# ERGO-Code/ipx

Hardware: AMD Instinct MI355X
Metric: kkt_solves_per_sec (higher is better)
Workload: dtype f64; 1 GPU; C3 synthetic LP m=1000000 n=2000000 8 nnz/col (nnz=16000000), KKTSolverDiag::Solve = diag-precond CR to tol=0.3*sqrt(mu), scaling spread s=1; rows of AI partitioned over 1 GPU(s); errflag=0

## Files before the change

### ipx_amd/csrc/cr.hip

```cpp
#include <cmath>

#include "context.hpp"
#include "spmv_kernels.hpp"

namespace ipxk {

constexpr int kWindow = 2;

enum CrMode { kModePcrDiag = 0, kModePcrSmw = 1, kModePlain = 2 };

struct CrVecs {
    int m;
    double* lhs;
    double* residual;
    double* sresidual;
    double* step;
    double* Cstep;
    double* Cres;
    double* pCstep;
    const double* resscale;
    const double* diag;
};

__global__ __launch_bounds__(kBlock) void residual_init_kernel(int m, const double* __restrict__ rhs,
                                                               const double* __restrict__ sub,
                                                               const double* __restrict__ resscale,
                                                               double* __restrict__ out,
                                                               double* partial) {
    __shared__ double red[kBlock / 64 + 1];
    double mx = 0.0;
    for (int i = blockIdx.x * kBlock + threadIdx.x; i < m; i += gridDim.x * kBlock) {
        const double r = sub ? rhs[i] - sub[i] : rhs[i];
        out[i] = r;
        mx = MaxOp::apply(mx, fabs(resscale ? resscale[i] * r : r));
    }
    mx = block_reduce<MaxOp>(mx, red);
    if (threadIdx.x == 0) partial[blockIdx.x] = mx;
}

__global__ __launch_bounds__(kBlock) void cr_init_state_kernel(CrState* st, double tol, long long maxiter,
                                                               long long hist_cap, PartRef rsdot, int mode) {
    __shared__ double red[kBlock / 64 + 1];
    const double r = rsdot.p ? reduce_partials<SumOp>(rsdot, red) : 0.0;
    if (threadIdx.x == 0) {
        st->tol = tol;
        st->maxiter = maxiter;
        st->k_started = 0;
        st->k_finished = 0;
        st->cdot[0] = st->cdot[1] = 0.0;
        st->rps[0] = r;
        st->rps[1] = 0.0;
        st->resnorm = 0.0;
        st->iter = 0;
        st->errflag = 0;
        st->done = 0;
        st->hist_cap = hist_cap;
        st->diag_rps_old = st->diag_rps_new = 0.0;
        st->mode = mode;
    }
}

template <int MODE>
__global__ __launch_bounds__(kBlock) void cr_control_update_kernel(
    CrState* st, CrVecs v, PartRef res0, PartRef res1, PartRef pdot_ref, PartRef rsdot_ref,
    double* res_next0, double* res_next1, double* hist) {
    if (st->done) return;
    __shared__ double red[kBlock / 64 + 1];
    const long long k = st->k_finished;
    const bool writer = blockIdx.x == 0 && threadIdx.x == 0;
    int errflag = -1;
    double resnorm = st->resnorm;

    if (MODE != kModePlain && k > 0 && k % 5 == 0) {
        const double rsdot = reduce_partials<SumOp>(rsdot_ref, red);
        const long long c5 = k / 5;
        if (rsdot >= st->rps[(c5 - 1) & 1]) {
            errflag = 204;
            if (writer) { st->diag_rps_old = st->rps[(c5 - 1) & 1]; st->diag_rps_new = rsdot; }
        } else if (writer) st->rps[c5 & 1] = rsdot;
    }
    double alpha = 0.0;
    if (errflag < 0) {
        resnorm = reduce_partials<MaxOp>((k & 1) ? res1 : res0, red);
        if (writer && k < st->hist_cap) hist[k] = resnorm;
        const double cdot = st->cdot[k & 1];
        if (resnorm <= st->tol) errflag = 0;
        else if (k == st->maxiter) errflag = 201;
        else if (cdot <= 0.0) errflag = 202;
        else {
            const double pdot = reduce_partials<SumOp>(pdot_ref, red);
            if (MODE != kModePlain && pdot <= 0.0) errflag = 203;
            else {
                alpha = cdot / pdot;
                if (!isfinite(alpha)) errflag = 205;
            }
        }
    }
    if (errflag >= 0) {
        if (writer) {
            st->errflag = errflag;
            st->iter = k;
            st->resnorm = resnorm;
            st->done = 1;
        }
        return;
    }

    double mx = 0.0;
    for (int i = blockIdx.x * kBlock + threadIdx.x; i < v.m; i += gridDim.x * kBlock) {
        const double q = v.Cstep[i];
        v.lhs[i] += alpha * v.step[i];
        const double r = v.residual[i] - alpha * q;
        v.residual[i] = r;
        if (MODE == kModePcrDiag) v.sresidual[i] -= alpha * (q / v.diag[i]);
        if (MODE == kModePcrSmw) v.sresidual[i] -= alpha * v.pCstep[i];
        mx = MaxOp::apply(mx, fabs(v.resscale ? v.resscale[i] * r : r));
    }
    mx = block_reduce<MaxOp>(mx, red);
    if (threadIdx.x == 0) ((k & 1) ? res_next0 : res_next1)[blockIdx.x] = mx;
    if (writer) {
        st->k_started = k + 1;
        st->resnorm = resnorm;
    }
}

template <int MODE, bool INIT>
__global__ __launch_bounds__(kBlock) void cr_direction_kernel(CrState* st, CrVecs v, PartRef cdot_ref,
                                                              double* pdot_partial) {
    if (st->done) return;
    __shared__ double red[kBlock / 64 + 1];
    const long long k = INIT ? -1 : st->k_started - 1;
    const double cdotnew = reduce_partials<SumOp>(cdot_ref, red);
    const double beta = INIT ? 0.0 : cdotnew / st->cdot[k & 1];
    const double* src = MODE == kModePlain ? v.residual : v.sresidual;
    double acc = 0.0;
    for (int i = blockIdx.x * kBlock + threadIdx.x; i < v.m; i += gridDim.x * kBlock) {
        double p, q;
        if (INIT) {
            p = src[i];
            q = v.Cres[i];
        } else {
            p = src[i] + beta * v.step[i];
            q = v.Cres[i] + beta * v.Cstep[i];
        }
        v.step[i] = p;
        v.Cstep[i] = q;
        if (MODE == kModePcrDiag) acc += (q / v.diag[i]) * q;
        if (MODE == kModePlain) acc += q * q;
    }
    if (MODE != kModePcrSmw) {
        acc = block_reduce<SumOp>(acc, red);
        if (threadIdx.x == 0) pdot_partial[blockIdx.x] = acc;
    }
    if (blockIdx.x == 0 && threadIdx.x == 0) {
        st->cdot[(k + 1) & 1] = cdotnew;
        st->k_finished = k + 1;
    }
}

__global__ __launch_bounds__(kBlock) void finalize_scalar_kernel(PartRef ref, int op, double* out) {
    __shared__ double red[kBlock / 64 + 1];
    const double v = op == 1 ? reduce_partials<MaxOp>(ref, red)
                   : op == 2 ? reduce_partials<MinOp>(ref, red) : reduce_partials<SumOp>(ref, red);
    if (threadIdx.x == 0) *out = v;
}

__global__ void snapshot_done_kernel(const CrState* st, int* host_slot) {
    __hip_atomic_store(host_slot, st->done, __ATOMIC_RELAXED, __HIP_MEMORY_SCOPE_SYSTEM);
}
__global__ void cycle_flags_kernel(const CrState* st, double interrupt_flag, double* flags) {
    flags[0] = (double)st->done;
    flags[1] = interrupt_flag;
}
__global__ void snapshot_flags_kernel(const double* flags, int* host_done, int* host_interrupt) {
    __hip_atomic_store(host_interrupt, (int)flags[1], __ATOMIC_RELAXED, __HIP_MEMORY_SCOPE_SYSTEM);
    __hip_atomic_store(host_done, (int)flags[0], __ATOMIC_RELAXED, __HIP_MEMORY_SCOPE_SYSTEM);
}

constexpr int kDoneRing = kWindow + 2;

static void ensure_comm_buffers(Context* c) {
    if (c->comm_scalars.size() < 64) c->comm_scalars.resize(64);
    if (c->comm_send.size() < (size_t)kNumPartialSlots) {
        c->comm_send.resize(kNumPartialSlots);
        IPXK_HIP(hipMemsetAsync(c->comm_send.get(), 0, sizeof(double) * kNumPartialSlots, c->stream));
    }
    const size_t need = (size_t)c->nranks * kNumPartialSlots;
    if (c->comm_gather.size() < need) c->comm_gather.resize(need);
}

struct Pub {
    Context* c;
    bool multi;
    explicit Pub(Context* ctx) : c(ctx), multi(comm_rows(ctx)) { if (multi) ensure_comm_buffers(ctx); }
    PartRef ref(int slot, int nparts) const {
        if (!multi) return PartRef{c->part(slot), nparts, 1};
        return PartRef{c->comm_gather.get() + slot, c->nranks, kNumPartialSlots};
    }
    void publish(int slot0, int n0, int op0, int slot1 = -1, int n1 = 0, int op1 = 0) const {
        if (!multi) return;
        hipLaunchKernelGGL(finalize_scalar_kernel, dim3(1), dim3(kBlock), 0, c->stream,
                           PartRef{c->part(slot0), n0, 1}, op0, c->comm_send.get() + slot0);
        if (slot1 >= 0)
            hipLaunchKernelGGL(finalize_scalar_kernel, dim3(1), dim3(kBlock), 0, c->stream,
                               PartRef{c->part(slot1), n1, 1}, op1, c->comm_send.get() + slot1);
        comm_allgather(c, c->comm_send.get(), c->comm_gather.get(), kNumPartialSlots);
    }
};

PartRef publish_scalar(Context* c, int slot, int count, int op) {
    const Pub pub(c);
    pub.publish(slot, count, op);
    return pub.ref(slot, count);
}

PartRef allreduce_scalar(Context* c, int slot, int count, int op) {
    ensure_comm_buffers(c);
    double* out = c->comm_scalars.get() + 62;
    hipLaunchKernelGGL(finalize_scalar_kernel, dim3(1), dim3(kBlock), 0, c->stream,
                       PartRef{c->part(slot), count, 1}, op, out);
    if (op == 0) comm_allreduce_sum(c, out, 1);
    else if (op == 1) comm_allreduce_max(c, out, 1);
    else comm_allreduce_min(c, out, 1);
    return PartRef{out, 1, 1};
}

double reduce_partials_host(Context* c, int slot, int count, bool is_max) {
    ensure_comm_buffers(c);
    double* out = c->comm_scalars.get() + 63;
    hipLaunchKernelGGL(finalize_scalar_kernel, dim3(1), dim3(kBlock), 0, c->stream,
                       PartRef{c->part(slot), count, 1}, is_max ? 1 : 0, out);
    if (comm_rows(c)) {
        if (is_max) comm_allreduce_max(c, out, 1);
        else comm_allreduce_sum(c, out, 1);
    }
    double v = 0.0;
    IPXK_HIP(hipMemcpyAsync(&v, out, sizeof(double), hipMemcpyDeviceToHost, c->stream));
    IPXK_HIP(hipStreamSynchronize(c->stream));
    return v;
}

static void ensure_workspaces(Context* c) {
    const size_t m = (size_t)(c->m > 0 ? c->m : 1);
    if (c->v_residual.size() != m) {
        c->v_residual.resize(m); c->v_sresidual.resize(m); c->v_step.resize(m);
        c->v_Cstep.resize(m); c->v_Cres.resize(m); c->v_pCstep.resize(m);
    }
    if (c->partials.size() == 0) c->partials.resize((size_t)kNumPartialSlots * kPartialStride);
    if (c->state.size() == 0) c->state.resize(1);
    if (!c->h_state) IPXK_HIP(hipHostMalloc(reinterpret_cast<void**>(&c->h_state), sizeof(CrState)));
    if (!c->ev_a) { IPXK_HIP(hipEventCreate(&c->ev_a)); IPXK_HIP(hipEventCreate(&c->ev_b)); }
    if (!c->h_cycle_done) {
        IPXK_HIP(hipHostMalloc(reinterpret_cast<void**>(&c->h_cycle_done), 64 * sizeof(int), hipHostMallocMapped));
        IPXK_HIP(hipHostGetDevicePointer(reinterpret_cast<void**>(&c->d_cycle_done), c->h_cycle_done, 0));
    }
    while ((int)c->ev_window.size() < kWindow + 1) {
        hipEvent_t e;
        IPXK_HIP(hipEventCreateWithFlags(&e, hipEventDisableTiming));
        c->ev_window.push_back(e);
    }
}

struct CrOps {
    int mode;
    int (*applyC)(Context*, const double* rhs, double* lhs, const int* done);
};

static int applyC_normal(Context* c, const double* rhs, double* lhs, const int* done) {
    int np = 0;
    time_mark(c, kTimeOp, true);
    normal_apply_dev(c, c->W, rhs, lhs, &np, done);
    time_mark(c, kTimeOp, false);
    return np;
}
static int applyC_split(Context* c, const double* rhs, double* lhs, const int* done) {
    return split_apply_dev(c, rhs, lhs, done);
}

template <int MODE>
static CrResult run_cr(Context* c, const CrOps& ops, const double* rhs, double tol,
                       const double* resscale, ipxint maxiter, double* lhs, bool lhs_is_zero,
                       ipxk_interrupt_fn interrupt, void* user, double* hist_host, ipxint hist_cap,
                       ipxk_times* times) {
    ensure_workspaces(c);
    time_start(c, times);
    hipStream_t s = c->stream;
    const int m = (int)c->m;
    if (maxiter < 0) maxiter = (comm_active(c) ? c->m_global : c->m) + 100;
    if (hist_cap < 0) hist_cap = 0;
    if (!hist_host) hist_cap = 0;
    if (c->hist.size() < (size_t)hist_cap + 1) c->hist.resize((size_t)hist_cap + 1);
    CrState* st = c->state.get();
    int* done = &st->done;
    const int g = vec_grid(m);
    const Pub pub(c);
    for (int i = 0; i < 2 * kDoneRing; i++) c->h_cycle_done[i] = 0;
    const bool multi = comm_active(c);
    if (multi) ensure_comm_buffers(c);

    CrVecs v;
    v.m = m; v.lhs = lhs; v.residual = c->v_residual.get(); v.sresidual = c->v_sresidual.get();
    v.step = c->v_step.get(); v.Cstep = c->v_Cstep.get(); v.Cres = c->v_Cres.get();
    v.pCstep = c->v_pCstep.get(); v.resscale = resscale; v.diag = c->reord.in_use ? c->reord.diagonal.get() : c->diagonal.get();

    IPXK_HIP(hipEventRecord(c->ev_a, s));

    if (lhs_is_zero) {
        hipLaunchKernelGGL(residual_init_kernel, dim3(g), dim3(kBlock), 0, s, m, rhs,
                           (const double*)nullptr, resscale, v.residual, c->part(kPartRes0));
    } else {
        ops.applyC(c, lhs, v.Cres, nullptr);
        hipLaunchKernelGGL(residual_init_kernel, dim3(g), dim3(kBlock), 0, s, m, rhs,
                           (const double*)v.Cres, resscale, v.residual, c->part(kPartRes0));
    }
    int nrsdot = 0;
    if (MODE != kModePlain) nrsdot = diag_apply_dev(c, v.residual, v.sresidual, kPartRsdot, nullptr);
    if (MODE != kModePlain) pub.publish(kPartRes0, g, 1, kPartRsdot, nrsdot, 0);
    else pub.publish(kPartRes0, g, 1);
    const PartRef res0 = pub.ref(kPartRes0, g), res1 = pub.ref(kPartRes1, g);
    const PartRef rsdot = MODE != kModePlain ? pub.ref(kPartRsdot, nrsdot) : PartRef{nullptr, 0, 1};
    hipLaunchKernelGGL(cr_init_state_kernel, dim3(1), dim3(kBlock), 0, s, st, tol, (long long)maxiter,
                       (long long)hist_cap, rsdot, (int)MODE);
    const double* csrc = MODE == kModePlain ? v.residual : v.sresidual;
    int ncdot = ops.applyC(c, csrc, v.Cres, nullptr);
    pub.publish(kPartCdot, ncdot, 0);
    hipLaunchKernelGGL((cr_direction_kernel<MODE, true>), dim3(g), dim3(kBlock), 0, s, st, v,
                       pub.ref(kPartCdot, ncdot), c->part(kPartPdot));
    int npdot = g;
    if (MODE == kModePcrSmw) npdot = diag_apply_dev(c, v.Cstep, v.pCstep, kPartPdot, nullptr);
    pub.publish(kPartPdot, npdot, 0);
    const PartRef pdot_ref = pub.ref(kPartPdot, npdot);

    ipxint interrupt_flag = 0, my_interrupt = 0;
    bool agreed_done = false;
    for (long long cycle = 0;; cycle++) {
        const long long k0 = cycle * 5;
        if (k0 > maxiter) break;
        if (cycle >= kWindow) {
            const long long cw = cycle - kWindow;
            IPXK_HIP(hipEventSynchronize(c->ev_window[cw % (kWindow + 1)]));
            if (*(volatile int*)(c->h_cycle_done + cw % kDoneRing)) { agreed_done = true; break; }
            if (multi) {
                const int agreed = *(volatile int*)(c->h_cycle_done + kDoneRing + cw % kDoneRing);
                if (agreed != 0) { interrupt_flag = agreed; break; }
            }
        }
        if (interrupt && cycle > 0) {
            my_interrupt = interrupt(user);
            if (!multi && my_interrupt != 0) { interrupt_flag = my_interrupt; break; }
        }
        for (long long k = k0; k < k0 + 5 && k <= maxiter; k++) {
            hipLaunchKernelGGL((cr_control_update_kernel<MODE>), dim3(g), dim3(kBlock), 0, s, st, v,
                               res0, res1, pdot_ref, rsdot, c->part(kPartRes0), c->part(kPartRes1),
                               c->hist.get());
            ncdot = ops.applyC(c, csrc, v.Cres, done);
            pub.publish(kPartCdot, ncdot, 0, ((k + 1) & 1) ? kPartRes1 : kPartRes0, g, 1);
            hipLaunchKernelGGL((cr_direction_kernel<MODE, false>), dim3(g), dim3(kBlock), 0, s, st, v,
                               pub.ref(kPartCdot, ncdot), c->part(kPartPdot));
            if (MODE == kModePcrSmw) diag_apply_dev(c, v.Cstep, v.pCstep, kPartPdot, done);
            if (MODE != kModePlain && (k + 1) % 5 == 0) {
                diag_apply_dev(c, v.residual, v.sresidual, kPartRsdot, done);
                pub.publish(kPartPdot, npdot, 0, kPartRsdot, nrsdot, 0);
            } else {
                pub.publish(kPartPdot, npdot, 0);
            }
        }
        if (multi) {
            double* flags = c->comm_scalars.get() + 56;
            hipLaunchKernelGGL(cycle_flags_kernel, dim3(1), dim3(1), 0, s, st, (double)my_interrupt, flags);
            comm_allreduce_max(c, flags, 2);
            hipLaunchKernelGGL(snapshot_flags_kernel, dim3(1), dim3(1), 0, s, flags, c->d_cycle_done + cycle % kDoneRing,
                               c->d_cycle_done + kDoneRing + cycle % kDoneRing);
        } else {
            hipLaunchKernelGGL(snapshot_done_kernel, dim3(1), dim3(1), 0, s, st, c->d_cycle_done + cycle % kDoneRing);
        }
        IPXK_HIP(hipEventRecord(c->ev_window[cycle % (kWindow + 1)], s));
    }
    IPXK_HIP(hipEventRecord(c->ev_b, s));
    IPXK_HIP(hipMemcpyAsync(c->h_state, st, sizeof(CrState), hipMemcpyDeviceToHost, s));
    IPXK_HIP(hipStreamSynchronize(s));
    IPXK_HIP(hipGetLastError());
    comm_check(c);

    if (multi && agreed_done && !c->h_state->done)
        throw Error(IPXK_E_HIP, "ranks of a partitioned solve diverged (another rank finished the CR loop, this one did not)");
    CrResult res;
    if (c->h_state->done) {
        res.iter = c->h_state->iter;
        res.errflag = c->h_state->errflag;
    } else {
        res.iter = c->h_state->k_finished;
        res.errflag = interrupt_flag;
    }
    if (hist_cap > 0) {
        long long nh = c->h_state->done && c->h_state->errflag != 204 ? res.iter + 1 : res.iter;
        if (!c->h_state->done) nh = c->h_state->k_started;
        if (nh > hist_cap) nh = hist_cap;
        for (long long i = nh; i < hist_cap; i++) hist_host[i] = std::nan("");
        if (nh > 0) {
            c->hist.download(hist_host, (size_t)nh, s);
            IPXK_HIP(hipStreamSynchronize(s));
        }
    }
    if (times) {
        float ms = 0.f;
        IPXK_HIP(hipEventElapsedTime(&ms, c->ev_a, c->ev_b));
        times->cr = ms * 1e-3;
        time_collect(c, times);
    }
    return res;
}

__global__ __launch_bounds__(kBlock) void infnorm_partial_kernel(int m, const double* __restrict__ x, double* partial) {
    __shared__ double red[kBlock / 64 + 1];
    double mx = 0.0;
    for (int i = blockIdx.x * kBlock + threadIdx.x; i < m; i += gridDim.x * kBlock) mx = MaxOp::apply(mx, fabs(x[i]));
    mx = block_reduce<MaxOp>(mx, red);
    if (threadIdx.x == 0) partial[blockIdx.x] = mx;
}

void cr_diagnostics_dev(Context* c, ipxk_cr_diag* out) {
    *out = ipxk_cr_diag{};
    IPXK_REQUIRE(c->h_state != nullptr && c->state.size() > 0, "no CR run on this context yet");
    const CrState& st = *c->h_state;
    out->errflag = st.done ? st.errflag : 0;
    out->iter = st.done ? st.iter : st.k_finished;
    out->maxiter = st.maxiter;
    out->resnorm = st.resnorm;
    out->tol = st.tol;
    out->cdot = st.cdot[out->iter & 1];
    out->rps_old = st.diag_rps_old;
    out->rps_new = st.diag_rps_new;
    if (st.done && st.errflag == 202) {
        const int m = (int)c->m, g = vec_grid(m);
        auto norm = [&](const double* v) {
            hipLaunchKernelGGL(infnorm_partial_kernel, dim3(g), dim3(kBlock), 0, c->stream, m, v, c->part(kPartScratch));
            return reduce_partials_host(c, kPartScratch, g, true);
        };
        out->infnorm_residual = norm(c->v_residual.get());
        if (st.mode != kModePlain) out->infnorm_sresidual = norm(c->v_sresidual.get());
    }
}

CrResult pcr_solve_dev(Context* c, const double* rhs, double tol, const double* resscale,
                       ipxint maxiter, double* lhs, bool lhs_is_zero, ipxk_interrupt_fn interrupt,
                       void* user, double* hist_host, ipxint hist_cap, ipxk_times* times) {
    IPXK_REQUIRE(c->normal_prepared, "NormalMatrix not prepared");
    IPXK_REQUIRE(c->diag_factorized, "DiagonalPrecond not factorized");
    CrOps ops{c->kdense > 0 ? kModePcrSmw : kModePcrDiag, applyC_normal};
    if (c->kdense > 0)
        return run_cr<kModePcrSmw>(c, ops, rhs, tol, resscale, maxiter, lhs, lhs_is_zero, interrupt,
                                   user, hist_host, hist_cap, times);
    return run_cr<kModePcrDiag>(c, ops, rhs, tol, resscale, maxiter, lhs, lhs_is_zero, interrupt, user,
                                hist_host, hist_cap, times);
}

CrResult cr_solve_dev(Context* c, const double* rhs, double tol, const double* resscale,
                      ipxint maxiter, double* lhs, bool lhs_is_zero, ipxk_interrupt_fn interrupt,
                      void* user, double* hist_host, ipxint hist_cap, ipxk_times* times) {
    IPXK_REQUIRE(c->split != nullptr, "SplittedNormalMatrix not prepared");
    split_check_partition(c);
    CrOps ops{kModePlain, applyC_split};
    return run_cr<kModePlain>(c, ops, rhs, tol, resscale, maxiter, lhs, lhs_is_zero, interrupt, user,
                              hist_host, hist_cap, times);
}

}
```

### ipx_amd/csrc/internal.hpp

```cpp
#pragma once

#include <hip/hip_runtime.h>

#include <chrono>
#include <cstdint>
#include <cstdio>
#include <cstdlib>
#include <algorithm>
#include <cstring>
#include <functional>
#include <memory>
#include <stdexcept>
#include <string>
#include <type_traits>
#include <vector>

#include "../../include/ipx_kkt_hip.h"

namespace ipxk {

struct Error : std::runtime_error {
    int code;
    Error(int c, const std::string& what) : std::runtime_error(what), code(c) {}
};

void set_last_error(const std::string& msg);

#define IPXK_HIP(expr)                                                         \
    do {                                                                       \
        hipError_t e_ = (expr);                                                \
        if (e_ != hipSuccess) {                                                \
            char buf_[512];                                                    \
            snprintf(buf_, sizeof buf_, "%s:%d: %s failed: %s", __FILE__,      \
                     __LINE__, #expr, hipGetErrorString(e_));                  \
            throw ::ipxk::Error(e_ == hipErrorOutOfMemory ? IPXK_E_ALLOC       \
                                                          : IPXK_E_HIP, buf_); \
        }                                                                      \
    } while (0)

#define IPXK_REQUIRE(cond, msg)                                                \
    do {                                                                       \
        if (!(cond))                                                           \
            throw ::ipxk::Error(IPXK_E_ARGUMENT, std::string(__func__) + ": " + (msg)); \
    } while (0)

void staged_h2d(void* dst_dev, const void* src_host, size_t bytes, hipStream_t s);
void staged_d2h(void* dst_host, const void* src_dev, size_t bytes, hipStream_t s);

template <class T>
class DevBuf {
public:
    DevBuf() = default;
    explicit DevBuf(size_t n) { resize(n); }
    DevBuf(const DevBuf&) = delete;
    DevBuf& operator=(const DevBuf&) = delete;
    DevBuf(DevBuf&& o) noexcept : p_(o.p_), n_(o.n_) { o.p_ = nullptr; o.n_ = 0; }
    DevBuf& operator=(DevBuf&& o) noexcept {
        if (this != &o) { release(); p_ = o.p_; n_ = o.n_; o.p_ = nullptr; o.n_ = 0; }
        return *this;
    }
    ~DevBuf() { release(); }
    void resize(size_t n) {
        if (n == n_) return;
        release();
        if (n > 0) IPXK_HIP(hipMalloc(reinterpret_cast<void**>(&p_), n * sizeof(T)));
        if (n > 0 && std::is_same<T, double>::value) {
            static const bool poison = getenv("IPXK_POISON") != nullptr;
            if (poison) { IPXK_HIP(hipMemset(p_, 0xff, n * sizeof(T))); IPXK_HIP(hipDeviceSynchronize()); }
        }
        n_ = n;
    }
    void ensure(size_t n) { if (n > n_) resize(n); }
    void release() {
        if (p_) (void)hipFree(p_);
        p_ = nullptr;
        n_ = 0;
    }
    T* get() const { return p_; }
    size_t size() const { return n_; }
    void upload(const T* host, size_t n, hipStream_t s) {
        if (n > n_) resize(n);
        if (n) staged_h2d(p_, host, n * sizeof(T), s);
    }
    void upload(const std::vector<T>& v, hipStream_t s) { upload(v.data(), v.size(), s); }
    void download(T* host, size_t n, hipStream_t s) const {
        if (n) staged_d2h(host, p_, n * sizeof(T), s);
    }
private:
    T* p_ = nullptr;
    size_t n_ = 0;
};

constexpr int kBlock = 256;
constexpr int kChunkNnz = 1024;
constexpr int kMaxRowLen = 255;
constexpr int kLongSeg = 2048;
constexpr int kMaxWorkgroups = 1024;
constexpr int kMaxPartials = 2048;
constexpr int kMaxRT = 8;

inline int grid_for(int64_t n, int cap = 4096) {
    int64_t g = (n + kBlock - 1) / kBlock;
    if (g < 1) g = 1;
    return (int)(g < cap ? g : cap);
}
inline int vec_grid(int64_t len) { return grid_for(len, 1024); }

struct GatherView {
    int nrows, ncols;
    int P, G, RT, Q;
    int RWrows;
    const int* step_ptr;
    const int* wg_chunk_ptr;
    const int* chunk_start;
    const int* chunk_info;
    const int* chunk_step;
    const unsigned char* counts;
    const int* idx;
    const double* val;
    const unsigned char* row_long;
    int nseg;
    const int* seg_p0;
    const int* seg_p1;
    const int* lidx;
    const double* lval;
    int nlong;
    const int* long_row;
    const int* long_slot;
    double* long_partials;
    unsigned long long* stamps;
    int masked;
};

constexpr int kSlicedRows = 1024;
constexpr int kSlicedMaxTile = 7680;

struct SlicedView {
    int nrows, nrows_pad, nslices, nrb;
    int R;
    const unsigned* tile_ptr;
    const unsigned char* cnt;
    const int* idx;
    const double* val;
    double* partial;
    const unsigned char* row_long;
    int masked;
};

struct SlicedMatrix {
    bool built = false;
    int nslices = 0, nrb = 0, nrows_pad = 0, max_tile = 0, R = kSlicedRows;
    double dominant_fraction = 1.0;
    DevBuf<unsigned> tile_ptr;
    DevBuf<unsigned char> cnt;
    DevBuf<int> idx;
    DevBuf<double> val, partial;
};

constexpr int kSortedThreads = 256;
constexpr int kSortedMaxSub = 8192;
constexpr int kSortedOffBits = 18;
struct SortedView {
    int nrows, nrows_pad, nslices, nsub, nrb, RB, slice_elems;
    const int* xmin;
    const unsigned char* row_long;
    const unsigned* sub_ptr;
    const unsigned char* cnt;
    const unsigned* pack;
    const double* val;
    double* partial;
};
struct SortedMatrix {
    bool built = false;
    int nslices = 0, nsub = 0, nrb = 0, RB = 0, nrows_pad = 0, max_sub = 0, slice_elems = 0;
    DevBuf<unsigned> sub_ptr, pack;
    DevBuf<unsigned char> cnt;
    DevBuf<double> val, partial;
    bool fused = false;
    DevBuf<int> xmin;
};

constexpr int kAccThreads = 512;
constexpr int kAccPerThread = 4;
constexpr int kAccBatch = kAccThreads * kAccPerThread;
constexpr int kAccMaxRows = 16384;
struct AccView {
    int nrows, nrows_pad, nslices, nrb, RB, slice_elems;
    const int* xmin;
    const unsigned* tile_batch;
    const unsigned* bptr;
    const unsigned* pack;
    const double* val;
    double* partial;
};
struct AccMatrix {
    bool built = false;
    int nslices = 0, nrb = 0, RB = 0, nrows_pad = 0, slice_elems = 0;
    int64_t nbatches = 0, deferred = 0;
    DevBuf<unsigned> tile_batch, bptr, pack;
    DevBuf<double> val, partial;
    bool fused = false;
    DevBuf<int> xmin;
};

struct LayoutScratch;

enum class SpmvLayout { phased, sliced, fused, sorted, sortedfused, acc, plain, accfused };
constexpr int kNumSpmvLayouts = 8;
inline constexpr const char* kSpmvLayoutNames[kNumSpmvLayouts] = {"phased", "sliced", "fused", "sorted", "sortedfused", "acc", "plain",
                                                                  "accfused"};

struct GatherMatrix {
    int nrows = 0, ncols = 0;
    int64_t nnz = 0;
    int P = 1, G = 1, RT = 1, Q = 1, RWrows = kBlock;
    DevBuf<int> step_ptr, idx, wg_chunk_ptr, chunk_start, chunk_info, chunk_step;
    DevBuf<unsigned char> counts, row_long;
    DevBuf<double> val;
    int nseg = 0, nlong = 0;
    DevBuf<int> seg_p0, seg_p1, lidx, long_row, long_slot;
    DevBuf<double> lval, long_partials;
    DevBuf<unsigned long long> stamps;
    int tune_level = 2;
    bool keep_plain = false;
    std::vector<int> h_plain_ptr;
    DevBuf<int> plain_idx;
    DevBuf<double> plain_val;

    void build(int64_t nrows_, int64_t ncols_, const ipxint* hptr, const ipxint* hidx,
               const double* hval, hipStream_t s);
    bool build_device(LayoutScratch& S, int64_t nrows_, int64_t ncols_, int64_t nnz_, const int* dptr, const int* didx,
                      const double* dval, hipStream_t s);
    bool build_device_local(LayoutScratch& S, int64_t nrows_, int64_t ncols_, int64_t nnz_, const int* dptr, const int* didx,
                            const double* dval, double share, hipStream_t s);
    void set_geometry(int64_t nrows_, int64_t ncols_);
    SpmvLayout layout = SpmvLayout::phased;
    SpmvLayout tile_base() const { return !sliced.built ? SpmvLayout::phased : sliced.nslices == 1 ? SpmvLayout::fused : SpmvLayout::sliced; }
    float tuned_us[kNumSpmvLayouts] = {};
    float time_layout(SpmvLayout L, hipStream_t s);
    void select_layout(const std::function<bool(SpmvLayout)>& make, hipStream_t s);
    SlicedMatrix sliced;
    SortedMatrix sorted;
    void build_sorted(const ipxint* hptr, const ipxint* hidx, const double* hval, hipStream_t s);
    void build_sorted_fused(const ipxint* hptr, const ipxint* hidx, const double* hval, hipStream_t s);
    AccMatrix acc;
    void build_acc(const ipxint* hptr, const ipxint* hidx, const double* hval, hipStream_t s);
    void build_acc_fused(const ipxint* hptr, const ipxint* hidx, const double* hval, hipStream_t s);
    AccMatrix accf;
    AccView acc_fused_view() const;
    AccView acc_view() const;
    const int* csr_ptr = nullptr;
    const int* csr_idx = nullptr;
    const double* csr_val = nullptr;
    int plain_grid() const { return (int)std::min<int64_t>(kMaxPartials, std::max<int64_t>(1, ((int64_t)nrows * 8 + kBlock - 1) / kBlock)); }
    int sorted_fused_grid() const {
        static const int cap = [] { const char* e = getenv("IPXK_SF_GRID"); return e && atoi(e) > 0 ? std::min(atoi(e), kMaxPartials) : kMaxPartials; }();
        return std::min(sorted.nrb, cap);
    }
    SortedView sorted_view() const;
    void build_sliced(const ipxint* hptr, const ipxint* hidx, const double* hval, hipStream_t s, int ns_request);
    SlicedView sliced_view(int which = 0) const;
    int fused_grid() const { return std::min(sliced.nrb, kMaxPartials); }
    int combine_grid() const { return (int)std::min<int64_t>(1024, std::max<int64_t>(1, ((int64_t)nrows + kBlock - 1) / kBlock)); }

    GatherView view(bool masked = false) const;
    int grid() const { return G; }
    DevBuf<double> valM, lvalM;
    struct CompactTiles {
        bool valid = false;
        DevBuf<unsigned> tile_ptr, tile_kept;
        DevBuf<unsigned char> cnt;
        DevBuf<int> idx;
        DevBuf<double> val;
    } compact;
    void compact_tiles(const double* weight, bool by_row, hipStream_t s);
    DevBuf<int> rowof;
    void mask_values(const double* weight, bool by_row, hipStream_t s);
    int num_partials(bool masked = false) const {
        int n;
        switch (masked ? tile_base() : layout) {
            case SpmvLayout::phased: n = G; break;
            case SpmvLayout::fused: n = fused_grid(); break;
            case SpmvLayout::sortedfused: n = sorted_fused_grid(); break;
            case SpmvLayout::plain: n = plain_grid(); break;
            case SpmvLayout::accfused: n = accf.nrb; break;
            default: n = combine_grid(); break;
        }
        return n + (nlong > 0 ? 1 : 0);
    }
    std::vector<unsigned char> h_row_long;
};

int slice_elems();
int64_t phase_slice(int64_t ncols);

struct CrState {
    double tol;
    long long maxiter;
    long long k_started;
    long long k_finished;
    double cdot[2];
    double rps[2];
    double resnorm;
    long long iter;
    int errflag;
    int done;
    long long hist_cap;
    double diag_rps_old, diag_rps_new;
    int mode;
};

struct MvScalars {
    int jn;
    double weight;
    int pmax, jb;
    double vmax, weight_recomp, colscale_jn, invscale_pmax, pivot_col;
    int used_pmax, eta_nnz;
    double pivot_row;
    int eta_total;
};

template <int kBest>
struct Partial { double v[kBest]; int i[kBest]; double s; int c; };
using MvPart = Partial<1>;

struct MaxvolState {
    DevBuf<double> colscale, invscale, colweights, row, mask, rhs, lhs, unit, btran, work;
    DevBuf<int> map2basis, slice_of, flag, rank, eta_ptr, eta_pos, eta_idx;
    DevBuf<double> eta_piv, eta_val;
    DevBuf<double> etaE, etaT, etaTt, eta_alpha, eta_d;
    DevBuf<int> eta_prev, eta_next, eta_last;
    DevBuf<double> etaF, etaG, eta_w;
    DevBuf<int> eta_first, eta_jof;
    DevBuf<ipxint> basis, status;
    DevBuf<MvPart> part;
    DevBuf<MvScalars> scalars;
    DevBuf<unsigned char> tmp;
    MvScalars* h = nullptr;
    struct Saved {
        bool live = false, dense = false, have_history = false;
        int K = 0, cap = 0, m = 0;
        int64_t sparse_used = 0, seg_nnz = 0;
        double overhead_s = 0.0, refactor_s = 0.0;
        long lu_generation = -1;
        int Kd = 0;
    } saved;
    std::vector<ipxint> basis_h;
    ~MaxvolState() { if (h) (void)hipHostFree(h); }
};

struct Context;

struct EtaFile {
    Context* c;
    MaxvolState& M;
    int m;
    hipStream_t s;
    bool dense = false, dense_possible = false, adaptive = false;
    int cap = 100;
    int limit = 100;
    int64_t sparse_cap = 0, sparse_used = 0;
    int K = 0;
    double overhead_s = 0.0, refactor_s = 0.0;
    int64_t seg_nnz = 0;
    bool have_history = false;
    bool resumed = false;

    double cost_list(double nnz) const { return 2.5e-6 + 0.5e-9 * nnz; }
    double cost_dense() const { return 0.6e-6 + 8.0 * (double)m / 2e12; }

    EtaFile(Context* ctx, MaxvolState& state, int rows, ipxint max_etas_in, bool resume = false);
    void save();
    bool worth_keeping() const;
    void reset(int block_rows);
    void append(const MvScalars* S, const double* lhs, int eta_nnz);
    bool full() const;
    void apply(bool transposed, double* v);
    static void apply_etas(MaxvolState& M, int m, int K, int cap, bool dense, bool transposed, double* v, hipStream_t s, int Kd = 0);
};

struct DeviceBasis {
    Context* c;
    MaxvolState& M;
    const int m;
    EtaFile etas;
    double& pivottol;
    std::vector<ipxint> basis_h, status_h;
    const double* colscale;
    MvScalars* S;
    double *rhs, *lhs, *unit, *btran;
    int64_t refused = 0, factorizations = 0, singular = 0;
    ipxint errflag = 0;

    DeviceBasis(Context* ctx, MaxvolState& state, ipxint max_etas, bool resume, const double* colscale_in, MvScalars* scalars);
    void ftran();
    void btran_unit();
    bool refactorize();
    bool exchange_if_stable(const MvScalars& a);
    void commit(const MvScalars& a);
};

template <class T>
T read_scalars(const T* dev, T* pinned, hipStream_t s) {
    IPXK_HIP(hipMemcpyAsync(pinned, dev, sizeof(T), hipMemcpyDeviceToHost, s));
    IPXK_HIP(hipStreamSynchronize(s));
    return *pinned;
}

inline double now_s() { return std::chrono::duration<double>(std::chrono::steady_clock::now().time_since_epoch()).count(); }

}

#include "layout_geometry.hpp"
```

Before: 56.25 solves/s.

## Defer lhs update into direction kernel, unroll CR vector loops, early-stop host enqueue

New measurement: 57.29 solves/s, median of 6. +1.9%, better.

```diff
diff --git a/ipx_amd/csrc/cr.hip b/ipx_amd/csrc/cr.hip
--- a/ipx_amd/csrc/cr.hip
+++ b/ipx_amd/csrc/cr.hip
@@ -8,6 +8,8 @@
 constexpr int kWindow = 2;
 
 enum CrMode { kModePcrDiag = 0, kModePcrSmw = 1, kModePlain = 2 };
+
+constexpr int kCrUnroll = 4;
 
 struct CrVecs {
     int m;
@@ -57,13 +59,15 @@
         st->hist_cap = hist_cap;
         st->diag_rps_old = st->diag_rps_new = 0.0;
         st->mode = mode;
+        st->alpha_pending = 0.0;
+        st->k_pending = -1;
     }
 }
 
 template <int MODE>
 __global__ __launch_bounds__(kBlock) void cr_control_update_kernel(
     CrState* st, CrVecs v, PartRef res0, PartRef res1, PartRef pdot_ref, PartRef rsdot_ref,
-    double* res_next0, double* res_next1, double* hist) {
+    double* res_next0, double* res_next1, double* hist, int lazy, int* host_done) {
     if (st->done) return;
     __shared__ double red[kBlock / 64 + 1];
     const long long k = st->k_finished;
@@ -102,25 +106,45 @@
             st->iter = k;
             st->resnorm = resnorm;
             st->done = 1;
+            if (host_done) __hip_atomic_store(host_done, 1, __ATOMIC_RELAXED, __HIP_MEMORY_SCOPE_SYSTEM);
         }
         return;
     }
 
     double mx = 0.0;
-    for (int i = blockIdx.x * kBlock + threadIdx.x; i < v.m; i += gridDim.x * kBlock) {
-        const double q = v.Cstep[i];
-        v.lhs[i] += alpha * v.step[i];
-        const double r = v.residual[i] - alpha * q;
-        v.residual[i] = r;
-        if (MODE == kModePcrDiag) v.sresidual[i] -= alpha * (q / v.diag[i]);
-        if (MODE == kModePcrSmw) v.sresidual[i] -= alpha * v.pCstep[i];
-        mx = MaxOp::apply(mx, fabs(v.resscale ? v.resscale[i] * r : r));
+    const long long stride = (long long)gridDim.x * kBlock, last = v.m - 1;
+    for (long long i0 = blockIdx.x * kBlock + threadIdx.x; i0 < v.m; i0 += kCrUnroll * stride) {
+        double q[kCrUnroll], r[kCrUnroll], sr[kCrUnroll] = {}, d[kCrUnroll] = {}, sc[kCrUnroll] = {};
+        double s[kCrUnroll] = {}, l[kCrUnroll] = {};
+#pragma unroll
+        for (int u = 0; u < kCrUnroll; u++) {
+            const long long i = min(i0 + u * stride, last);
+            q[u] = v.Cstep[i];
+            r[u] = v.residual[i];
+            if (MODE != kModePlain) sr[u] = v.sresidual[i];
+            if (MODE == kModePcrDiag) d[u] = v.diag[i];
+            if (MODE == kModePcrSmw) d[u] = v.pCstep[i];
+            if (v.resscale) sc[u] = v.resscale[i];
+            if (!lazy) { s[u] = v.step[i]; l[u] = v.lhs[i]; }
+        }
+#pragma unroll
+        for (int u = 0; u < kCrUnroll; u++) {
+            const long long i = i0 + u * stride;
+            if (i > last) break;
+            if (!lazy) v.lhs[i] = l[u] + alpha * s[u];
+            const double rn = r[u] - alpha * q[u];
+            v.residual[i] = rn;
+            if (MODE == kModePcrDiag) v.sresidual[i] = sr[u] - alpha * (q[u] / d[u]);
+            if (MODE == kModePcrSmw) v.sresidual[i] = sr[u] - alpha * d[u];
+            mx = MaxOp::apply(mx, fabs(v.resscale ? sc[u] * rn : rn));
+        }
     }
     mx = block_reduce<MaxOp>(mx, red);
     if (threadIdx.x == 0) ((k & 1) ? res_next0 : res_next1)[blockIdx.x] = mx;
     if (writer) {
         st->k_started = k + 1;
         st->resnorm = resnorm;
+        if (lazy) { st->alpha_pending = alpha; st->k_pending = k; }
     }
 }
 
@@ -133,20 +157,35 @@
     const double cdotnew = reduce_partials<SumOp>(cdot_ref, red);
     const double beta = INIT ? 0.0 : cdotnew / st->cdot[k & 1];
     const double* src = MODE == kModePlain ? v.residual : v.sresidual;
+    const bool owed = !INIT && st->k_pending == k;
+    const double alpha = st->alpha_pending;
     double acc = 0.0;
-    for (int i = blockIdx.x * kBlock + threadIdx.x; i < v.m; i += gridDim.x * kBlock) {
-        double p, q;
-        if (INIT) {
-            p = src[i];
-            q = v.Cres[i];
-        } else {
-            p = src[i] + beta * v.step[i];
-            q = v.Cres[i] + beta * v.Cstep[i];
-        }
-        v.step[i] = p;
-        v.Cstep[i] = q;
-        if (MODE == kModePcrDiag) acc += (q / v.diag[i]) * q;
-        if (MODE == kModePlain) acc += q * q;
+    const long long stride = (long long)gridDim.x * kBlock, last = v.m - 1;
+    for (long long i0 = blockIdx.x * kBlock + threadIdx.x; i0 < v.m; i0 += kCrUnroll * stride) {
+        double p[kCrUnroll], q[kCrUnroll], s[kCrUnroll] = {}, cs[kCrUnroll] = {}, d[kCrUnroll] = {}, l[kCrUnroll] = {};
+#pragma unroll
+        for (int u = 0; u < kCrUnroll; u++) {
+            const long long i = min(i0 + u * stride, last);
+            p[u] = src[i];
+            q[u] = v.Cres[i];
+            if (!INIT) { s[u] = v.step[i]; cs[u] = v.Cstep[i]; }
+            if (MODE == kModePcrDiag) d[u] = v.diag[i];
+            if (owed) l[u] = v.lhs[i];
+        }
+#pragma unroll
+        for (int u = 0; u < kCrUnroll; u++) {
+            const long long i = i0 + u * stride;
+            if (i > last) break;
+            if (!INIT) {
+                if (owed) v.lhs[i] = l[u] + alpha * s[u];
+                p[u] = p[u] + beta * s[u];
+                q[u] = q[u] + beta * cs[u];
+            }
+            v.step[i] = p[u];
+            v.Cstep[i] = q[u];
+            if (MODE == kModePcrDiag) acc += (q[u] / d[u]) * q[u];
+            if (MODE == kModePlain) acc += q[u] * q[u];
+        }
     }
     if (MODE != kModePcrSmw) {
         acc = block_reduce<SumOp>(acc, red);
@@ -156,6 +195,12 @@
         st->cdot[(k + 1) & 1] = cdotnew;
         st->k_finished = k + 1;
     }
+}
+
+__global__ __launch_bounds__(kBlock) void cr_flush_update_kernel(const CrState* st, CrVecs v) {
+    if (st->k_pending < 0 || st->k_pending != st->k_finished) return;
+    const double alpha = st->alpha_pending;
+    for (int i = blockIdx.x * kBlock + threadIdx.x; i < v.m; i += gridDim.x * kBlock) v.lhs[i] += alpha * v.step[i];
 }
 
 __global__ __launch_bounds__(kBlock) void finalize_scalar_kernel(PartRef ref, int op, double* out) {
@@ -178,6 +223,12 @@
 }
 
 constexpr int kDoneRing = kWindow + 2;
+constexpr int kDoneNow = 2 * kDoneRing;
+
+static bool cr_lazy() {
+    static const bool setting = [] { const char* e = getenv("IPXK_CR_LAZY"); return !e || atoi(e) != 0; }();
+    return setting;
+}
 
 static void ensure_comm_buffers(Context* c) {
     if (c->comm_scalars.size() < 64) c->comm_scalars.resize(64);
@@ -294,8 +345,10 @@
     int* done = &st->done;
     const int g = vec_grid(m);
     const Pub pub(c);
-    for (int i = 0; i < 2 * kDoneRing; i++) c->h_cycle_done[i] = 0;
+    for (int i = 0; i <= kDoneNow; i++) c->h_cycle_done[i] = 0;
     const bool multi = comm_active(c);
+    const int lazy = cr_lazy() ? 1 : 0;
+    int* done_now = multi ? nullptr : c->d_cycle_done + kDoneNow;
     if (multi) ensure_comm_buffers(c);
 
     CrVecs v;
@@ -332,7 +385,7 @@
     const PartRef pdot_ref = pub.ref(kPartPdot, npdot);
 
     ipxint interrupt_flag = 0, my_interrupt = 0;
-    bool agreed_done = false;
+    bool agreed_done = false, tail = false;
     for (long long cycle = 0;; cycle++) {
         const long long k0 = cycle * 5;
         if (k0 > maxiter) break;
@@ -350,9 +403,11 @@
             if (!multi && my_interrupt != 0) { interrupt_flag = my_interrupt; break; }
         }
         for (long long k = k0; k < k0 + 5 && k <= maxiter; k++) {
+            if (done_now && *(volatile int*)(c->h_cycle_done + kDoneNow)) tail = true;
+            if (tail) break;
             hipLaunchKernelGGL((cr_control_update_kernel<MODE>), dim3(g), dim3(kBlock), 0, s, st, v,
                                res0, res1, pdot_ref, rsdot, c->part(kPartRes0), c->part(kPartRes1),
-                               c->hist.get());
+                               c->hist.get(), lazy, done_now);
             ncdot = ops.applyC(c, csrc, v.Cres, done);
             pub.publish(kPartCdot, ncdot, 0, ((k + 1) & 1) ? kPartRes1 : kPartRes0, g, 1);
             hipLaunchKernelGGL((cr_direction_kernel<MODE, false>), dim3(g), dim3(kBlock), 0, s, st, v,
@@ -376,6 +431,7 @@
         }
         IPXK_HIP(hipEventRecord(c->ev_window[cycle % (kWindow + 1)], s));
     }
+    if (lazy) hipLaunchKernelGGL(cr_flush_update_kernel, dim3(g), dim3(kBlock), 0, s, st, v);
     IPXK_HIP(hipEventRecord(c->ev_b, s));
     IPXK_HIP(hipMemcpyAsync(c->h_state, st, sizeof(CrState), hipMemcpyDeviceToHost, s));
     IPXK_HIP(hipStreamSynchronize(s));
diff --git a/ipx_amd/csrc/internal.hpp b/ipx_amd/csrc/internal.hpp
--- a/ipx_amd/csrc/internal.hpp
+++ b/ipx_amd/csrc/internal.hpp
@@ -308,6 +308,8 @@
     long long hist_cap;
     double diag_rps_old, diag_rps_new;
     int mode;
+    double alpha_pending;
+    long long k_pending;
 };
 
 struct MvScalars {
```
